# swyoon/Diffusion-by-MaxEntIRL

Hardware: AMD Instinct MI355X
Metric: images/sec (CIFAR-10 DDPM T=10 generation) (higher is better)
Workload: dtype bf16

## Files before the change

diffusion-by-maxentirl_amd/csrc/conv1x1_rw.hip:

```cpp
#include "conv_common.h"
#include <stdlib.h>

namespace {

#define RW_GPTR(p) ((const __attribute__((address_space(1))) void*)(p))
#define RW_LPTR(p) ((__attribute__((address_space(3))) void*)(p))
#define RW_WAIT_VM(n) asm volatile("s_waitcnt vmcnt(%0)" ::"n"(n) : "memory")
__device__ __forceinline__ void rw_barrier() { asm volatile("s_waitcnt lgkmcnt(0)\n\ts_barrier" ::: "memory"); }

constexpr int RW_CHUNK = 64 * 256;
constexpr int RW_RO = 64 * 256;

template <int NCH, int R, bool RES>
__global__ __launch_bounds__(256, ((NCH > 3 || R > 4) ? 1 : 2)) void conv1x1_rw_kernel(ConvArgs p) {
    static_assert(R - 1 <= 4 * NCH && R >= 3 && 4 * (R - 2) + 4 * (RES ? 8 : 4) < 64, "ring depth");
    constexpr int BOPS = RES ? 8 : 4;
    constexpr int NYOUNG = 4 * (R - 2);
    extern __shared__ __attribute__((aligned(1024))) char smem[];
    char* const ring = smem;

    const int tid = threadIdx.x, lane = tid & 63, h = lane >> 5;
    const int wave = __builtin_amdgcn_readfirstlane(tid >> 6);
    char* const ro = smem + R * RW_CHUNK + wave * 4096;
    const int xcd = blockIdx.x & 7, j = blockIdx.x >> 3;
    const int cot = j % p.CT;
    const int nstreams = (gridDim.x >> 3) / p.CT * 8;
    const int stream = (j / p.CT) * 8 + xcd;
    const int ntiles = stream < p.PT ? (p.PT - stream + nstreams - 1) / nstreams : 0;
    if (ntiles == 0) return;

    bf16x8 A[NCH * 8];
    {
        const bf16x8* wf = reinterpret_cast<const bf16x8*>(p.w) + (size_t)(cot * 4 + wave) * 64 + lane;
#pragma unroll
        for (int ks = 0; ks < NCH * 8; ++ks) A[ks] = wf[(size_t)ks * p.CB * 64];
    }
    f32x4 bv[4];
#pragma unroll
// ... 5 lines not shown
    const float slope = dxmi_act_slope(p.act);

    int dpx[4], ds8[4];
#pragma unroll
    for (int u = 0; u < 4; ++u) {
        dpx[u] = (wave * 4 + u) * 4 + (lane >> 4);
        ds8[u] = ((lane & 15) ^ (dpx[u] & 15)) * 8;
    }
    auto issue_chunk = [&](int tile, int c, int slot) {
        const size_t P0 = (size_t)(stream + tile * nstreams) * 64;
        const int cbase = c * 128;
        const bool first = cbase < p.C0;
        const bf16* src = first ? p.in0 : p.in1;
        const int Cs = first ? p.C0 : p.C1;
        const int coff = first ? cbase : cbase - p.C0;
#pragma unroll
        for (int u = 0; u < 4; ++u)
            __builtin_amdgcn_global_load_lds(RW_GPTR(src + (P0 + dpx[u]) * Cs + coff + ds8[u]),
                                             RW_LPTR(ring + slot * RW_CHUNK + (wave * 4 + u) * 1024), 16, 0, 0);
    };
    int rpx[4], rc8[4];
#pragma unroll
    for (int i = 0; i < 4; ++i) {
        rpx[i] = i * 16 + (lane >> 2);
        rc8[i] = ((lane & 3) ^ ((rpx[i] >> 1) & 3)) * 8;
    }
    auto tile_off = [&](int tile, int i) -> size_t {
        return ((size_t)(stream + tile * nstreams) * 64 + rpx[i]) * p.Cout + cot * 128 + wave * 32 + rc8[i];
    };
    auto issue_residual = [&](int tile) {
// ... 3 lines not shown
    };

    const int gtot = ntiles * NCH;
    if (RES) issue_residual(0);
#pragma unroll
    for (int g = 0; g < R - 1; ++g)
        if (g < gtot) issue_chunk(g / NCH, g % NCH, g);

    int boff[8];
    {
        const int px = lane & 31;
#pragma unroll
        for (int ks = 0; ks < 8; ++ks) boff[ks] = px * 256 + (((ks * 2 + h) ^ (px & 15)) << 4);
    }

    int slot = 0;
    for (int ti = 0; ti < ntiles; ++ti) {
        f32x16 acc[2];
#pragma unroll
        for (int nb = 0; nb < 2; ++nb)
#pragma unroll
            for (int r = 0; r < 16; ++r) acc[nb][r] = 0.f;
#pragma unroll
        for (int c = 0; c < NCH; ++c) {
            const int g = ti * NCH + c;
            const int kmax = R - 1 - c > 0 ? (R - 1 - c + NCH - 1) / NCH : 0;
            const int nbnd = ti < kmax ? ti : kmax;
            if (g + R - 2 >= gtot) RW_WAIT_VM(0);
            else if (nbnd == 0) RW_WAIT_VM(NYOUNG);
            else if (nbnd == 1) RW_WAIT_VM(NYOUNG + BOPS);
            else if (nbnd == 2) RW_WAIT_VM(NYOUNG + 2 * BOPS);
            else if (nbnd == 3) RW_WAIT_VM(NYOUNG + 3 * BOPS);
            else RW_WAIT_VM(NYOUNG + 4 * BOPS);
            rw_barrier();
            {
                const int gi = g + R - 1;
                const int si = slot == 0 ? R - 1 : slot - 1;
                if (gi < gtot) issue_chunk(ti + (c + R - 1) / NCH, (c + R - 1) % NCH, si);
            }
            const char* img = ring + slot * RW_CHUNK;
#pragma unroll
            for (int ks = 0; ks < 8; ++ks)
#pragma unroll
                for (int nb = 0; nb < 2; ++nb) {
                    const bf16x8 b = *reinterpret_cast<const bf16x8*>(img + boff[ks] + nb * (32 * 256));
                    acc[nb] = __builtin_amdgcn_mfma_f32_32x32x16_bf16(A[c * 8 + ks], b, acc[nb], 0, 0, 0);
                }
            slot = slot + 1 == R ? 0 : slot + 1;
        }
        if (RES) {
            if ((ti + 1) * NCH + R - 1 > gtot) RW_WAIT_VM(0);
            else RW_WAIT_VM(4 * NCH);
        }
#pragma unroll
        for (int nb = 0; nb < 2; ++nb) {
            const int px = nb * 32 + (lane & 31);
#pragma unroll
            for (int g4 = 0; g4 < 4; ++g4) {
                char* a = ro + px * 64 + ((g4 ^ ((px >> 1) & 3)) << 4) + 8 * h;
                f32x4 v;
#pragma unroll
                for (int e = 0; e < 4; ++e) v[e] = acc[nb][4 * g4 + e] + bv[g4][e];
// ... 13 lines not shown
            bf16x8 v[4];
#pragma unroll
            for (int i = 0; i < 4; ++i) v[i] = *reinterpret_cast<const bf16x8*>(ro + i * 1024 + lane * 16);
#pragma unroll
            for (int i = 0; i < 4; ++i) *reinterpret_cast<bf16x8*>(reinterpret_cast<bf16*>(p.out) + tile_off(ti, i)) = v[i];
        }
        if (RES && ti + 1 < ntiles) issue_residual(ti + 1);
    }
}

template <int NCH, int R>
int rw_launch(const ConvArgs& b, int grid, hipStream_t st) {
    const size_t lds = (size_t)R * RW_CHUNK + RW_RO;
    static bool attr_set = false;
    if (!attr_set) {
        (void)hipFuncSetAttribute(reinterpret_cast<const void*>(conv1x1_rw_kernel<NCH, R, true>), hipFuncAttributeMaxDynamicSharedMemorySize, 160 * 1024);
        (void)hipFuncSetAttribute(reinterpret_cast<const void*>(conv1x1_rw_kernel<NCH, R, false>), hipFuncAttributeMaxDynamicSharedMemorySize, 160 * 1024);
        attr_set = true;
    }
    if (b.residual) hipLaunchKernelGGL((conv1x1_rw_kernel<NCH, R, true>), dim3(grid), dim3(256), lds, st, b);
    else hipLaunchKernelGGL((conv1x1_rw_kernel<NCH, R, false>), dim3(grid), dim3(256), lds, st, b);
    DXMI_CHECK_LAUNCH("dxmi_conv2d_fwd(1x1 rw)");
    return DXMI_OK;
}

}

int conv1x1_rw_try_launch(ConvArgs& a, hipStream_t st, int* kernel_id) {
    static const int enabled = getenv("DXMI_CONV1X1_RW") ? atoi(getenv("DXMI_CONV1X1_RW")) : 1;
    if (!enabled) return 1;
    if (a.in_mode != DXMI_IN_NHWC_BF16 || a.out_mode != DXMI_OUT_NHWC_BF16) return 1;
    if (a.ksize != 1 || a.stride != 1 || a.pad != 0 || a.ups != 0 || a.mask_src || a.addvec || a.act == DXMI_ACT_SILU) return 1;
    const int K = a.C0 + a.C1;
    if (K % 128 != 0 || a.C0 % 128 != 0 || K > 512 || a.Cout % 128 != 0) return 1;
    const long px = (long)a.N * a.OH * a.OW;
    if (px % 64 != 0 || px / 64 < 512) return 1;
    if (kernel_id) {
        const int nch = K / 128;
        *kernel_id = 500000 + nch * 1000 + (nch > 3 ? 6 : 3) * 10 + (a.residual ? 1 : 0);
        return DXMI_OK;
    }
    ConvArgs b = a;
    b.PT = (int)(px / 64);
    b.CT = a.Cout / 128;
    b.tile_px = 64;
    if (b.CT > 32) return 1;
    const int per_xcd = K > 384 ? 32 : 64;
    const int grid = 8 * b.CT * (per_xcd / b.CT);
    switch (K / 128) {
    case 1: return rw_launch<1, 3>(b, grid, st);
    case 2: return rw_launch<2, 3>(b, grid, st);
    case 3: return rw_launch<3, 3>(b, grid, st);
    default: return rw_launch<4, 6>(b, grid, st);
    }
}
```

diffusion-by-maxentirl_amd/csrc/groupnorm.hip:

```cpp
#include "conv_common.h"
#include <stdlib.h>

namespace {

__device__ __forceinline__ int xcd_logical_block(int b, int G, int on = 1) {
    if (!on) return b;
    const int x = b & 7, k = b >> 3;
    const int q = G >> 3, r = G & 7;
    return x * q + (x < r ? x : r) + k;
}

struct GnArgs {
    const bf16* in0;
    const bf16* in1;
    const float* gamma;
    const float* beta;
    bf16* out;
    int C0, C1, HW, groups, slices, ppp, cpg, gps;
    int xcd;
    float eps;
    int silu;
    int fast;
};

// ... 276 lines not shown
struct GnApplyArgs {
    const bf16* in0;
    const bf16* in1;
    const float* st0;
    const float* st1;
    const float* gamma;
    const float* beta;
    const float* ss;
    bf16* out;
    int C0, C1, HW, groups, cpg, chunks, rows_per_chunk, P0, P1, ss_ld;
    float eps;
    int silu;
    int nt;
    float* ab;
};

constexpr int GN_APPLY_MAXP = 8;

typedef int gn_i4 __attribute__((ext_vector_type(4)));
__device__ __forceinline__ bf16x8 gn_ld(const bf16* ptr, bool nt) {
    const gn_i4* q = reinterpret_cast<const gn_i4*>(ptr);
    const gn_i4 t = nt ? __builtin_nontemporal_load(q) : *q;
    return __builtin_bit_cast(bf16x8, t);
}
__device__ __forceinline__ void gn_st(bf16* ptr, const bf16x8& v, bool nt) {
    gn_i4* q = reinterpret_cast<gn_i4*>(ptr);
    const gn_i4 t = __builtin_bit_cast(gn_i4, v);
    if (nt) __builtin_nontemporal_store(t, q);
    else *q = t;
}

template <int U>
// ... 20 lines not shown
        for (int u = 0; u < U; ++u) {
            const int rr = r + u * rows_par;
            if (rr < row1) v[u] = gn_ld(src + (size_t)rr * Cs, p.nt & 1);
        }
    }
    float A[8], Bv[8];
    if (p.ab) {
        if (!active) return;
        const f32x4* q = reinterpret_cast<const f32x4*>(p.ab + ((size_t)n * C + c) * 2);
        const f32x4 t0 = q[0], t1 = q[1], t2 = q[2], t3 = q[3];
        A[0] = t0[0]; Bv[0] = t0[1]; A[1] = t0[2]; Bv[1] = t0[3];
        A[2] = t1[0]; Bv[2] = t1[1]; A[3] = t1[2]; Bv[3] = t1[3];
        A[4] = t2[0]; Bv[4] = t2[1]; A[5] = t2[2]; Bv[5] = t2[3];
        A[6] = t3[0]; Bv[6] = t3[1]; A[7] = t3[2]; Bv[7] = t3[3];
    } else {
    auto pair_sums = [&](const float* st, int P, int nbs, int off) {
        const float2* const base = reinterpret_cast<const float2*>(st) + (size_t)n * P * nbs;
        for (int b = tid; b < nbs; b += 256) {
            float2 t[GN_APPLY_MAXP];
#pragma unroll
            for (int k = 0; k < GN_APPLY_MAXP; ++k)
                if (k < P) t[k] = base[(unsigned)(k * nbs + b)];
            float s = 0.f, q = 0.f;
#pragma unroll
            for (int k = 0; k < GN_APPLY_MAXP; ++k)
                if (k < P) {
                    s += t[k].x;
                    q += t[k].y;
                }
            for (int k = GN_APPLY_MAXP; k < P; ++k) {
                const float2 tk = base[(unsigned)(k * nbs + b)];
                s += tk.x;
                q += tk.y;
            }
            pair_s[off + b] = make_float2(s, q);
        }
    };
    pair_sums(p.st0, p.P0, p.C0 >> 1, 0);
    if (p.C1) pair_sums(p.st1, p.P1, p.C1 >> 1, p.C0 >> 1);
    __syncthreads();
    f32x4 g0, g1, b0, b1;
    if (active) {
        g0 = *reinterpret_cast<const f32x4*>(p.gamma + c);
        g1 = *reinterpret_cast<const f32x4*>(p.gamma + c + 4);
        b0 = *reinterpret_cast<const f32x4*>(p.beta + c);
        b1 = *reinterpret_cast<const f32x4*>(p.beta + c + 4);
    }
    f32x4 sc0 = {0.f, 0.f, 0.f, 0.f}, sc1 = sc0, sh0 = sc0, sh1 = sc0;
    if (active && p.ss) {
        const float* ssn = p.ss + (size_t)n * p.ss_ld + c;
        sc0 = *reinterpret_cast<const f32x4*>(ssn);
        sc1 = *reinterpret_cast<const f32x4*>(ssn + 4);
        sh0 = *reinterpret_cast<const f32x4*>(ssn + C);
        sh1 = *reinterpret_cast<const f32x4*>(ssn + C + 4);
    }
    if (tid < p.groups) {
        const int bpg = p.cpg >> 1;
        float s = 0.f, q = 0.f;
        for (int b = tid * bpg; b < (tid + 1) * bpg; ++b) {
            s += pair_s[b].x;
            q += pair_s[b].y;
        }
        const float cnt = (float)p.HW * (float)p.cpg;
        const float m = s / cnt;
        mean_s[tid] = m;
        rstd_s[tid] = rsqrtf(fmaxf(q / cnt - m * m, 0.f) + p.eps);
    }
    __syncthreads();
    if (!active) return;
    {
#pragma unroll
        for (int e = 0; e < 8; ++e) {
            const int g = (c + e) / p.cpg;
            float a = rstd_s[g] * (e < 4 ? g0[e] : g1[e - 4]);
            float b = (e < 4 ? b0[e] : b1[e - 4]) - mean_s[g] * a;
            if (p.ss) {
                const float sc = 1.f + (e < 4 ? sc0[e] : sc1[e - 4]);
                a *= sc;
                b = b * sc + (e < 4 ? sh0[e] : sh1[e - 4]);
            }
            A[e] = a;
            Bv[e] = b;
        }
    }
    }
    for (;;) {
#pragma unroll
        for (int u = 0; u < U; ++u) {
            const int rr = r + u * rows_par;
            if (rr < row1) {
                bf16x8 o;
#pragma unroll
                for (int e = 0; e < 8; ++e) {
                    float y = (float)v[u][e] * A[e] + Bv[e];
                    if (p.silu) y = dxmi_silu_fast(y);
                    o[e] = (bf16)y;
                }
                gn_st(dst + (size_t)rr * C, o, p.nt & 2);
            }
        }
        r += U * rows_par;
        if (r >= row1) break;
#pragma unroll
        for (int u = 0; u < U; ++u) {
            const int rr = r + u * rows_par;
            if (rr < row1) v[u] = gn_ld(src + (size_t)rr * Cs, p.nt & 1);
        }
    }
}

__global__ __launch_bounds__(256) void gn_block_stats_kernel(const bf16* __restrict__ x, float* __restrict__ st, int HW, int C,
                                                             int chunks, int rows_per_chunk) {
    __shared__ float sm[256 * 8];
// ... 966 lines not shown

extern "C" int dxmi_groupnorm_generic_bwd(const void* in0, int32_t C0, const void* in1, int32_t C1, const void* dy,
                                          const void* add0, const void* add1, const float* gamma, const float* beta,
                                          const float* scale_shift, int32_t ss_ld, void* dx0, void* dx1, float* g_out,
                                          void* workspace, int32_t N, int32_t HW, int32_t groups, float eps,
                                          int32_t apply_silu, void* stream) {
    return dxmi_groupnorm_generic_bwd_saved(in0, C0, in1, C1, dy, add0, add1, gamma, beta, scale_shift, ss_ld, dx0, dx1, g_out, nullptr,
                                            workspace, N, HW, groups, eps, apply_silu, stream);
}

__global__ __launch_bounds__(256) void gn_finalize_kernel(GnApplyArgs p) {
    __shared__ float mean_s[32], rstd_s[32];
    __shared__ float2 pair_s[1024];
    const int C = p.C0 + p.C1;
    const int n = blockIdx.x, tid = threadIdx.x;
    auto pair_sums = [&](const float* st, int P, int nbs, int off) {
        const float2* const base = reinterpret_cast<const float2*>(st) + (size_t)n * P * nbs;
        for (int b = tid; b < nbs; b += 256) {
            float2 t[GN_APPLY_MAXP];
#pragma unroll
            for (int k = 0; k < GN_APPLY_MAXP; ++k)
                if (k < P) t[k] = base[(unsigned)(k * nbs + b)];
            float s = 0.f, q = 0.f;
#pragma unroll
            for (int k = 0; k < GN_APPLY_MAXP; ++k)
                if (k < P) {
                    s += t[k].x;
                    q += t[k].y;
                }
            for (int k = GN_APPLY_MAXP; k < P; ++k) {
                const float2 tk = base[(unsigned)(k * nbs + b)];
                s += tk.x;
                q += tk.y;
            }
            pair_s[off + b] = make_float2(s, q);
        }
    };
    pair_sums(p.st0, p.P0, p.C0 >> 1, 0);
    if (p.C1) pair_sums(p.st1, p.P1, p.C1 >> 1, p.C0 >> 1);
    __syncthreads();
    if (tid < p.groups) {
        const int bpg = p.cpg >> 1;
        float s = 0.f, q = 0.f;
        for (int b = tid * bpg; b < (tid + 1) * bpg; ++b) {
            s += pair_s[b].x;
            q += pair_s[b].y;
        }
        const float cnt = (float)p.HW * (float)p.cpg;
        const float m = s / cnt;
        mean_s[tid] = m;
        rstd_s[tid] = rsqrtf(fmaxf(q / cnt - m * m, 0.f) + p.eps);
    }
    __syncthreads();
    for (int c = tid; c < C; c += 256) {
        const int g = c / p.cpg;
        float a = rstd_s[g] * p.gamma[c];
        float b = p.beta[c] - mean_s[g] * a;
        if (p.ss) {
            const float sc = 1.f + p.ss[(size_t)n * p.ss_ld + c];
            a *= sc;
            b = b * sc + p.ss[(size_t)n * p.ss_ld + C + c];
        }
        reinterpret_cast<float2*>(p.ab)[(size_t)n * C + c] = make_float2(a, b);
    }
}

__global__ __launch_bounds__(256) void gn_blockstats_to_generic_kernel(const float* __restrict__ st0, int P0, int C0, const float* __restrict__ st1,
                                                                      int P1, int C1, float* __restrict__ part, int groups, int chunks) {
    __shared__ float2 pair_s[1024];
    const int n = blockIdx.x, tid = threadIdx.x;
    const int C = C0 + C1, cpg = C / groups;
    auto pair_sums = [&](const float* st, int P, int nbs, int off) {
        const float2* const base = reinterpret_cast<const float2*>(st) + (size_t)n * P * nbs;
        for (int b = tid; b < nbs; b += 256) {
            float s = 0.f, q = 0.f;
            for (int k = 0; k < P; ++k) {
                const float2 t = base[(size_t)k * nbs + b];
// ... 144 lines not shown
    int rpc = trips_env * U * rows_par;
    if (rpc > HW) rpc = HW;
    a.chunks = (HW + rpc - 1) / rpc;
    a.rows_per_chunk = rpc;
    a.ab = ab;
    if (ab) {
        hipLaunchKernelGGL(gn_finalize_kernel, dim3(N), dim3(256), 0, (hipStream_t)stream, a);
        DXMI_CHECK_LAUNCH("dxmi_groupnorm_apply_split(finalize)");
    }
    if (U == 8) hipLaunchKernelGGL(gn_apply_kernel<8>, dim3(N * a.chunks), dim3(256), 0, (hipStream_t)stream, a);
    else if (U == 2) hipLaunchKernelGGL(gn_apply_kernel<2>, dim3(N * a.chunks), dim3(256), 0, (hipStream_t)stream, a);
    else hipLaunchKernelGGL(gn_apply_kernel<4>, dim3(N * a.chunks), dim3(256), 0, (hipStream_t)stream, a);
    DXMI_CHECK_LAUNCH("dxmi_groupnorm_apply");
    return DXMI_OK;
}
```

diffusion-by-maxentirl_amd/dxmi_hip/_lib.py:

```python
import ctypes
import os

_HERE = os.path.dirname(os.path.abspath(__file__))
LIB_PATH = os.environ.get("DXMI_LIB") or os.path.join(_HERE, "libdxmi_hip.so")

c_void_p, c_int, c_float, c_int64 = ctypes.c_void_p, ctypes.c_int32, ctypes.c_float, ctypes.c_int64


class ConvDesc(ctypes.Structure):

    _fields_ = [
        ("in0", c_void_p), ("in1", c_void_p), ("wpacked", c_void_p), ("bias", c_void_p),
        ("addvec", c_void_p), ("residual", c_void_p), ("out", c_void_p),
        ("N", c_int), ("IH", c_int), ("IW", c_int), ("C0", c_int), ("C1", c_int),
        ("OH", c_int), ("OW", c_int), ("Cout", c_int),
        ("ksize", c_int), ("stride", c_int), ("pad", c_int), ("upsample", c_int), ("act", c_int),
        ("addvec_ld", c_int), ("in_mode", c_int), ("out_mode", c_int), ("variant", c_int),
        ("mask_src", c_void_p), ("mask_slope", c_float), ("gn_stats", c_void_p),
        ("gn_out", c_void_p), ("gn_gamma", c_void_p), ("gn_beta", c_void_p), ("gn_eps", c_float), ("gn_groups", c_int), ("gn_flags", c_int),
    ]


class PackItem(ctypes.Structure):

# ... 7 lines not shown
    "dxmi_device_check": (c_int, []),
    "dxmi_set_tuning": (c_int, [ctypes.c_char_p, c_int]),
    "dxmi_get_tuning": (c_int, [ctypes.c_char_p, ctypes.POINTER(c_int)]),
    "dxmi_conv2d_fwd": (c_int, [ctypes.POINTER(ConvDesc), c_void_p]),
    "dxmi_conv2d_kernel_id": (c_int, [ctypes.POINTER(ConvDesc)]),
    "dxmi_conv2d_gn_stats_partials": (c_int, [ctypes.POINTER(ConvDesc)]),
    "dxmi_conv2d_gn_fuse_supported": (c_int, [ctypes.POINTER(ConvDesc)]),
    "dxmi_conv_ws_last_clock": (c_int, [ctypes.POINTER(ctypes.c_uint64)]),
    "dxmi_gn_block_stats_partials": (c_int, [c_int]),
    "dxmi_gn_block_stats": (c_int, [c_void_p, c_void_p, c_int, c_int, c_int, c_void_p]),
    "dxmi_gn_stats_fold": (c_int, [c_void_p, c_void_p, c_int, c_int, c_int, c_int, c_void_p]),
    "dxmi_groupnorm_apply": (c_int, [c_void_p, c_int, c_void_p, c_int, c_void_p, c_int, c_void_p, c_int, c_void_p, c_void_p, c_void_p, c_int,
                                     c_void_p, c_int, c_int, c_int, c_float, c_int, c_void_p]),
    "dxmi_groupnorm_apply_split": (c_int, [c_void_p, c_int, c_void_p, c_int, c_void_p, c_int, c_void_p, c_int, c_void_p, c_void_p, c_void_p, c_int,
                                           c_void_p, c_void_p, c_int, c_int, c_int, c_float, c_int, c_void_p]),
    "dxmi_gn_blockstats_to_generic": (c_int, [c_void_p, c_int, c_int, c_void_p, c_int, c_int, c_void_p, c_int, c_int, c_int, c_void_p]),
    "dxmi_attention_fwd_lse_supported": (c_int, [c_int, c_int, c_int]),
    "dxmi_attention_fwd_lse": (c_int, [c_void_p, c_void_p, c_void_p, c_int, c_int, c_int, c_int, c_float, c_void_p]),
    "dxmi_attention_bwd_lse": (c_int, [c_void_p, c_void_p, c_void_p, c_void_p, c_void_p, c_void_p, c_int, c_int, c_int, c_int, c_float, c_void_p]),
    "dxmi_gn_ss_grads": (c_int, [c_void_p, c_void_p, c_int, c_void_p, c_void_p, c_void_p, c_void_p, c_void_p, c_int, c_int, c_void_p]),
    "dxmi_fid_stats_workspace_bytes": (c_int64, [c_int64, c_int]),
    "dxmi_fid_stats": (c_int, [c_void_p, c_int64, c_int, c_void_p, c_void_p, c_void_p, c_void_p]),
    "dxmi_knn_radii_workspace_bytes": (c_int64, [c_int64, c_int, c_int, c_int]),
    "dxmi_knn_radii": (c_int, [c_void_p, c_int64, c_int, c_int, c_int, c_void_p, c_void_p, c_void_p]),
    "dxmi_pr_membership_workspace_bytes": (c_int64, [c_int64, c_int64]),
    "dxmi_pr_membership": (c_int, [c_void_p, c_int64, c_void_p, c_void_p, c_int64, c_void_p, c_int, c_void_p, c_void_p, c_void_p, c_void_p]),
    "dxmi_inception_score_workspace_bytes": (c_int64, [c_int64, c_int, c_int]),
    "dxmi_inception_score": (c_int, [c_void_p, c_int64, c_int, c_void_p, c_int, c_int, c_void_p, c_void_p, c_void_p]),
    "dxmi_packed_conv_weight_bytes": (c_int64, [c_int, c_int, c_int, c_int]),
    "dxmi_pack_conv_weights": (c_int, [ctypes.POINTER(PackItem), c_int, c_void_p]),
# ... 102 lines not shown
```

diffusion-by-maxentirl_amd/dxmi_hip/ops.py:

```python
import ctypes
import os

import torch

from . import _lib
from . import graph as _graph
from ._lib import ConvDesc, check, load

ACT_NONE, ACT_LEAKY02, ACT_RELU, ACT_SILU = 0, 1, 2, 3
IN_NHWC_BF16, IN_NCHW_F32_K27 = 0, 1
OUT_NHWC_BF16, OUT_NCHW_F32 = 0, 1


_RAW_STREAM = getattr(torch._C, "_cuda_getCurrentRawStream", None)
_GET_DEVICE = getattr(torch._C, "_cuda_getDevice", None)


def _stream():
    if _RAW_STREAM is not None and _GET_DEVICE is not None:
        return ctypes.c_void_p(_RAW_STREAM(_GET_DEVICE()))
    return ctypes.c_void_p(torch.cuda.current_stream().cuda_stream)


def _tree_fingerprint(module):
# ... 664 lines not shown
            saved.append(gn_blockstats_to_generic(stats[0], stats[1] if in1 is not None else None, N, H * W, C0, C1, groups))
        return groupnorm_apply(x, stats[0], gamma, beta, in1=in1, st1=stats[1] if in1 is not None else None, groups=groups,
                               eps=eps, silu=silu, out=out, scale_shift=scale_shift)
    if scale_shift is not None or not load().dxmi_groupnorm_silu_supported(C0, C1, H * W, groups):
        return groupnorm_generic(x, gamma, beta, in1=in1, groups=groups, eps=eps, silu=silu, out=out, scale_shift=scale_shift, saved=saved)
    assert x.dtype == torch.bfloat16 and x.is_contiguous()
    assert gamma.dtype == torch.float32 and beta.dtype == torch.float32 and gamma.numel() == C0 + C1
    if out is None:
        out = torch.empty((N, H, W, C0 + C1), dtype=torch.bfloat16, device=x.device)
    _prof("groupnorm", "resident", 0.0, 4.0 * N * H * W * (C0 + C1), lambda: check(
        load().dxmi_groupnorm_silu_fwd(_ptr(x), C0, _ptr(in1), C1, _ptr(gamma), _ptr(beta), _ptr(out), N, H * W,
                                       groups, float(eps), int(silu), _stream()), "dxmi_groupnorm_silu_fwd"))
    return out


def gn_blockstats_to_generic(st0, st1, N, HW, C0, C1, groups=32):
    lib = load()
    ws = torch.empty(lib.dxmi_groupnorm_generic_workspace_bytes(N, HW, C0 + C1) // 4, dtype=torch.float32, device=st0.buf.device)
    check(lib.dxmi_gn_blockstats_to_generic(_ptr(st0.buf), st0.P, C0, _ptr(st1.buf) if st1 is not None else None, st1.P if st1 is not None else 0,
                                            C1, _ptr(ws), N, HW, groups, _stream()), "dxmi_gn_blockstats_to_generic")
    return ws


def groupnorm_generic(x, gamma, beta, *, in1=None, groups=32, eps=1e-5, silu=True, out=None, scale_shift=None, saved=None):
    _need_cuda(x, in1, gamma, beta, out, scale_shift)
    N, H, W, C0 = x.shape
    C1 = in1.shape[3] if in1 is not None else 0
    C = C0 + C1
    assert x.dtype == torch.bfloat16 and x.is_contiguous()
    if out is None:
# ... 616 lines not shown
```

diffusion-by-maxentirl_amd/models/DxMI/unet_small.py:

```python
import torch
import torch.nn as nn

from dxmi_hip import ops
from dxmi_hip._lib import DxmiError


def Normalize(in_channels):
    return nn.GroupNorm(num_groups=32, num_channels=in_channels, eps=1e-6, affine=True)


def _conv(cin, cout, k, stride=1, padding=0):
    return nn.Conv2d(cin, cout, kernel_size=k, stride=stride, padding=padding)


class Upsample(nn.Module):

    def __init__(self, in_channels, with_conv):
        super().__init__()
        self.with_conv = with_conv
        if with_conv:
            self.conv = _conv(in_channels, in_channels, 3, 1, 1)


class Downsample(nn.Module):
# ... 183 lines not shown
        return self._packed

    def refresh_packs(self):
        self.packed()
        if getattr(self, "_packed_t", None) is not None:
            from .unet_small_train import _pack_t
            _pack_t(self)

    def prepare_capture(self):
        if getattr(self, "_packed_t", None) is not None:
            for k in [k for k in self._packed_t if k not in self._packed_t_planned]:
                del self._packed_t[k]
        self.refresh_packs()

    FUSE_ATTN_PROJ = True
    FUSE_ATTN_BLOCK = True
    FUSE_GN_SMALL = True
    STREAM_GN_MIN_HW = 256

    def _conv_s(self, x, pw, **kw):
        out, st = ops.conv2d(x, pw, want_stats=True, **kw)
        if st is None and out.shape[1] * out.shape[2] >= self.STREAM_GN_MIN_HW:
            st = ops.block_stats(out)
        return out, st

    def _resblock(self, pk, b, x0, x1, tp, s0=None, s1=None, nxt=None):
        if isinstance(s0, _Normed):
            assert s0.norm is b.norm1 and x1 is None
            a0 = s0.y
        else:
            a0 = ops.groupnorm_silu(x0, b.norm1.weight, b.norm1.bias, in1=x1, eps=1e-6, silu=True, stats=(s0, s1))
        off = pk[id(b), "toff"]
        stream = x0.shape[1] * x0.shape[2] >= self.STREAM_GN_MIN_HW
        a = None
        if not stream and self.FUSE_GN_SMALL:
            h, a = ops.conv2d(a0, pk[id(b), "conv1"], bias=b.conv1.bias, addvec=tp[:, off:off + b.out_channels],
                              fuse_gn=(b.norm2.weight, b.norm2.bias, 32, 1e-6, True, False))
            sh = None
            if a is None and stream:
                sh = ops.block_stats(h)
        else:
            h, sh = ops.conv2d(a0, pk[id(b), "conv1"], bias=b.conv1.bias, addvec=tp[:, off:off + b.out_channels], want_stats=True)
        if a is None:
            a = ops.groupnorm_silu(h, b.norm2.weight, b.norm2.bias, eps=1e-6, silu=True, stats=(sh, None))
        if b.in_channels != b.out_channels:
            sc_mod = b.conv_shortcut if b.use_conv_shortcut else b.nin_shortcut
            sc = ops.conv2d(x0, pk[id(b), "short"], in1=x1, bias=sc_mod.bias)
        else:
            assert x1 is None
            sc = x0
        if stream:
            return self._conv_s(a, pk[id(b), "conv2"], bias=b.conv2.bias, residual=sc)
        if nxt is not None and self.FUSE_GN_SMALL:
            h, y = ops.conv2d(a, pk[id(b), "conv2"], bias=b.conv2.bias, residual=sc,
                              fuse_gn=(nxt[0].weight, nxt[0].bias, 32, 1e-6, nxt[1], True))
            return h, (None if y is None else _Normed(y, nxt[0]))
        return ops.conv2d(a, pk[id(b), "conv2"], bias=b.conv2.bias, residual=sc), None

    def _attn(self, pk, m, x, sx=None):
        N, H, W, C = x.shape
        if self.FUSE_ATTN_BLOCK and (id(m), "block") in pk and isinstance(sx, ops.BlockStats) and ops.attn_block_supported(H * W, C, 1):
            return ops.attn_block(x, sx, m.norm.weight, m.norm.bias, pk[id(m), "block"], eps=1e-6, want_stats=True)
# ... 98 lines not shown
```

include/dxmi_hip.h:

```cpp
#ifndef DXMI_HIP_H
#define DXMI_HIP_H

#include <stdint.h>

#ifdef __cplusplus
extern "C" {
#endif

#define DXMI_OK            0
#define DXMI_EINVAL       -1
#define DXMI_ELAUNCH      -2
#define DXMI_ENODEV       -3

#define DXMI_ACT_NONE      0
#define DXMI_ACT_LEAKY02   1
#define DXMI_ACT_RELU      2
#define DXMI_ACT_SILU      3

#define DXMI_IN_NHWC_BF16     0
#define DXMI_IN_NCHW_F32_K27  1
#define DXMI_IN_ROWS_F32      2
#define DXMI_OUT_NHWC_BF16    0
#define DXMI_OUT_NCHW_F32     1
#define DXMI_OUT_ROWS_F32     2
// ... 115 lines not shown
                            int32_t apply_silu, void* stream);

int dxmi_gn_block_stats_partials(int32_t HW);
int dxmi_gn_block_stats(const void* x, float* stats, int32_t N, int32_t HW, int32_t C, void* stream);
int dxmi_gn_stats_fold(const float* stats, float* out, int32_t N, int32_t P, int32_t C, int32_t group, void* stream);
int dxmi_groupnorm_apply(const void* in0, int32_t C0, const float* stats0, int32_t P0, const void* in1, int32_t C1,
                         const float* stats1, int32_t P1, const float* gamma, const float* beta, const float* scale_shift,
                         int32_t ss_ld, void* out, int32_t N, int32_t HW, int32_t groups, float eps, int32_t apply_silu,
                         void* stream);

int dxmi_groupnorm_apply_split(const void* in0, int32_t C0, const float* stats0, int32_t P0, const void* in1, int32_t C1,
                               const float* stats1, int32_t P1, const float* gamma, const float* beta,
                               const float* scale_shift, int32_t ss_ld, void* out, float* ab_workspace, int32_t N, int32_t HW,
                               int32_t groups, float eps, int32_t apply_silu, void* stream);

int dxmi_gn_blockstats_to_generic(const float* stats0, int32_t P0, int32_t C0, const float* stats1, int32_t P1, int32_t C1,
                                  float* generic_stats, int32_t N, int32_t HW, int32_t groups, void* stream);

int dxmi_gn_ss_grads(const float* g, const float* scale_shift, int32_t ss_ld, const float* gamma, const float* beta,
                     float* d_scale_shift, float* dgamma, float* dbeta, int32_t N, int32_t C, void* stream);

int dxmi_attention_fwd(const void* qkv, void* out, int32_t N, int32_t T, int32_t C,
                       int32_t heads, float scale, void* stream);

int dxmi_attention_proj_supported(int32_t T, int32_t C, int32_t heads);
int dxmi_pack_attn_proj_weight(const float* w_oi, void* dst, void* stream);
int dxmi_attention_proj_fwd(const void* qkv, const void* wproj_packed, const float* bias, const void* residual, void* out,
                            float* gn_stats, int32_t N, int32_t T, int32_t C, int32_t heads, float scale, void* stream);

int dxmi_attn_block_supported(int32_t T, int32_t C, int32_t heads, int32_t groups);
// ... 188 lines not shown
```

Baseline: 6733.

## Fuse GroupNorm+SiLU apply into the 1x1 shortcut conv kernel

Adds a GN variant of the 1x1 streaming conv kernel. While computing the nin_shortcut it normalizes the staged input chunks already in LDS and writes the GroupNorm+SiLU output as a side result. Per-image scale/shift tables are loaded into LDS alongside each chunk, and vmcnt waits are recomputed through a runtime switch. The resblock path uses it when channels change at large spatial sizes, so the input is read once instead of twice. The cost is an extra gn_finalize launch, more LDS, extra stores inside the MFMA loop, and more complex wait-count bookkeeping.

```diff
diff --git a/diffusion-by-maxentirl_amd/csrc/conv1x1_rw.hip b/diffusion-by-maxentirl_amd/csrc/conv1x1_rw.hip
--- a/diffusion-by-maxentirl_amd/csrc/conv1x1_rw.hip
+++ b/diffusion-by-maxentirl_amd/csrc/conv1x1_rw.hip
@@ -1,4 +1,5 @@
 #include "conv_common.h"
+#include "gn_common.h"
 #include <stdlib.h>
 
 namespace {
@@ -10,10 +11,29 @@
 
 constexpr int RW_CHUNK = 64 * 256;
 constexpr int RW_RO = 64 * 256;
-
-template <int NCH, int R, bool RES>
-__global__ __launch_bounds__(256, ((NCH > 3 || R > 4) ? 1 : 2)) void conv1x1_rw_kernel(ConvArgs p) {
+constexpr int RW_TBL = 128 * 8;
+
+struct RwGn {
+    const float* ab;
+    bf16* y;
+    int HW, silu;
+};
+
+__device__ __forceinline__ void rw_wait_vm(int n) {
+    switch (__builtin_amdgcn_readfirstlane(n)) {
+#define RW_C(k) case k: RW_WAIT_VM(k); break;
+#define RW_C8(k) RW_C(k) RW_C(k + 1) RW_C(k + 2) RW_C(k + 3) RW_C(k + 4) RW_C(k + 5) RW_C(k + 6) RW_C(k + 7)
+    RW_C8(0) RW_C8(8) RW_C8(16) RW_C8(24) RW_C8(32) RW_C8(40) RW_C8(48) RW_C8(56)
+#undef RW_C8
+#undef RW_C
+    default: RW_WAIT_VM(0);
+    }
+}
+
+template <int NCH, int R, bool RES, bool GN>
+__global__ __launch_bounds__(256, ((NCH > 3 || R > 4) ? 1 : 2)) void conv1x1_rw_kernel(ConvArgs p, RwGn q) {
     static_assert(R - 1 <= 4 * NCH && R >= 3 && 4 * (R - 2) + 4 * (RES ? 8 : 4) < 64, "ring depth");
+    static_assert(!(GN && RES) && (!GN || 5 * (R - 2) + 4 * 4 + 4 * (R - 1) < 64), "GN side output: no residual, vmcnt range");
     constexpr int BOPS = RES ? 8 : 4;
     constexpr int NYOUNG = 4 * (R - 2);
     extern __shared__ __attribute__((aligned(1024))) char smem[];
@@ -22,6 +42,7 @@
     const int tid = threadIdx.x, lane = tid & 63, h = lane >> 5;
     const int wave = __builtin_amdgcn_readfirstlane(tid >> 6);
     char* const ro = smem + R * RW_CHUNK + wave * 4096;
+    char* const tbl = smem + R * RW_CHUNK + RW_RO;
     const int xcd = blockIdx.x & 7, j = blockIdx.x >> 3;
     const int cot = j % p.CT;
     const int nstreams = (gridDim.x >> 3) / p.CT * 8;
@@ -57,6 +78,11 @@
         const bf16* src = first ? p.in0 : p.in1;
         const int Cs = first ? p.C0 : p.C1;
         const int coff = first ? cbase : cbase - p.C0;
+        if constexpr (GN) {
+            const int n = (int)P0 / q.HW;
+            __builtin_amdgcn_global_load_lds(RW_GPTR(q.ab + ((size_t)n * (NCH * 128) + cbase) * 2 + wave * 64 + lane),
+                                             RW_LPTR(tbl + slot * RW_TBL + wave * 256), 4, 0, 0);
+        }
 #pragma unroll
         for (int u = 0; u < 4; ++u)
             __builtin_amdgcn_global_load_lds(RW_GPTR(src + (P0 + dpx[u]) * Cs + coff + ds8[u]),
@@ -90,6 +116,9 @@
         for (int ks = 0; ks < 8; ++ks) boff[ks] = px * 256 + (((ks * 2 + h) ^ (px & 15)) << 4);
     }
 
+    const int gnp = GN ? 4 / p.CT : 0;
+    const int gs = tid & 15, gpx0 = cot * (64 / p.CT) + (tid >> 4);
+
     int slot = 0;
     for (int ti = 0; ti < ntiles; ++ti) {
         f32x16 acc[2];
@@ -103,6 +132,7 @@
             const int kmax = R - 1 - c > 0 ? (R - 1 - c + NCH - 1) / NCH : 0;
             const int nbnd = ti < kmax ? ti : kmax;
             if (g + R - 2 >= gtot) RW_WAIT_VM(0);
+            else if (GN) rw_wait_vm(5 * (R - 2) + nbnd * BOPS + (g < R - 1 ? g : R - 1) * gnp);
             else if (nbnd == 0) RW_WAIT_VM(NYOUNG);
             else if (nbnd == 1) RW_WAIT_VM(NYOUNG + BOPS);
             else if (nbnd == 2) RW_WAIT_VM(NYOUNG + 2 * BOPS);
@@ -122,6 +152,21 @@
                     const bf16x8 b = *reinterpret_cast<const bf16x8*>(img + boff[ks] + nb * (32 * 256));
                     acc[nb] = __builtin_amdgcn_mfma_f32_32x32x16_bf16(A[c * 8 + ks], b, acc[nb], 0, 0, 0);
                 }
+            if constexpr (GN) {
+                float ga[8], gb[8];
+                const f32x4* t = reinterpret_cast<const f32x4*>(tbl + slot * RW_TBL + gs * 64);
+#pragma unroll
+                for (int i = 0; i < 4; ++i) {
+                    const f32x4 v = t[i];
+                    ga[2 * i] = v[0]; gb[2 * i] = v[1]; ga[2 * i + 1] = v[2]; gb[2 * i + 1] = v[3];
+                }
+                bf16* const yt = q.y + (size_t)(stream + ti * nstreams) * 64 * (NCH * 128) + c * 128 + gs * 8;
+                for (int i = 0; i < gnp; ++i) {
+                    const int px = gpx0 + 16 * i;
+                    const bf16x8 v = *reinterpret_cast<const bf16x8*>(img + px * 256 + ((gs ^ (px & 15)) << 4));
+                    *reinterpret_cast<bf16x8*>(yt + (size_t)px * (NCH * 128)) = gn_norm8(v, ga, gb, q.silu);
+                }
+            }
             slot = slot + 1 == R ? 0 : slot + 1;
         }
         if (RES) {
@@ -165,14 +210,37 @@
     const size_t lds = (size_t)R * RW_CHUNK + RW_RO;
     static bool attr_set = false;
     if (!attr_set) {
-        (void)hipFuncSetAttribute(reinterpret_cast<const void*>(conv1x1_rw_kernel<NCH, R, true>), hipFuncAttributeMaxDynamicSharedMemorySize, 160 * 1024);
-        (void)hipFuncSetAttribute(reinterpret_cast<const void*>(conv1x1_rw_kernel<NCH, R, false>), hipFuncAttributeMaxDynamicSharedMemorySize, 160 * 1024);
+        (void)hipFuncSetAttribute(reinterpret_cast<const void*>(conv1x1_rw_kernel<NCH, R, true, false>), hipFuncAttributeMaxDynamicSharedMemorySize, 160 * 1024);
+        (void)hipFuncSetAttribute(reinterpret_cast<const void*>(conv1x1_rw_kernel<NCH, R, false, false>), hipFuncAttributeMaxDynamicSharedMemorySize, 160 * 1024);
         attr_set = true;
     }
-    if (b.residual) hipLaunchKernelGGL((conv1x1_rw_kernel<NCH, R, true>), dim3(grid), dim3(256), lds, st, b);
-    else hipLaunchKernelGGL((conv1x1_rw_kernel<NCH, R, false>), dim3(grid), dim3(256), lds, st, b);
+    const RwGn none = {};
+    if (b.residual) hipLaunchKernelGGL((conv1x1_rw_kernel<NCH, R, true, false>), dim3(grid), dim3(256), lds, st, b, none);
+    else hipLaunchKernelGGL((conv1x1_rw_kernel<NCH, R, false, false>), dim3(grid), dim3(256), lds, st, b, none);
     DXMI_CHECK_LAUNCH("dxmi_conv2d_fwd(1x1 rw)");
     return DXMI_OK;
+}
+
+template <int NCH, int R>
+int rw_launch_gn(const ConvArgs& b, const RwGn& g, int grid, hipStream_t st) {
+    const size_t lds = (size_t)R * (RW_CHUNK + RW_TBL) + RW_RO;
+    static bool attr_set = false;
+    if (!attr_set) {
+        (void)hipFuncSetAttribute(reinterpret_cast<const void*>(conv1x1_rw_kernel<NCH, R, false, true>), hipFuncAttributeMaxDynamicSharedMemorySize, 160 * 1024);
+        attr_set = true;
+    }
+    hipLaunchKernelGGL((conv1x1_rw_kernel<NCH, R, false, true>), dim3(grid), dim3(256), lds, st, b, g);
+    DXMI_CHECK_LAUNCH("dxmi_groupnorm_silu_shortcut");
+    return DXMI_OK;
+}
+
+int rw_grid(ConvArgs& b) {
+    const int K = b.C0 + b.C1;
+    b.PT = (int)((long)b.N * b.OH * b.OW / 64);
+    b.CT = b.Cout / 128;
+    b.tile_px = 64;
+    const int per_xcd = K > 384 ? 32 : 64;
+    return 8 * b.CT * (per_xcd / b.CT);
 }
 
 }
@@ -192,12 +260,8 @@
         return DXMI_OK;
     }
     ConvArgs b = a;
-    b.PT = (int)(px / 64);
-    b.CT = a.Cout / 128;
-    b.tile_px = 64;
-    if (b.CT > 32) return 1;
-    const int per_xcd = K > 384 ? 32 : 64;
-    const int grid = 8 * b.CT * (per_xcd / b.CT);
+    if (a.Cout / 128 > 32) return 1;
+    const int grid = rw_grid(b);
     switch (K / 128) {
     case 1: return rw_launch<1, 3>(b, grid, st);
     case 2: return rw_launch<2, 3>(b, grid, st);
@@ -205,3 +269,48 @@
     default: return rw_launch<4, 6>(b, grid, st);
     }
 }
+
+static int gn_shortcut_nch(const dxmi_conv_desc* d, int groups) {
+    if (!d || d->ksize != 1 || d->stride != 1 || d->pad != 0 || d->upsample || d->residual || d->addvec || d->mask_src || d->gn_stats ||
+        d->gn_out || d->act != DXMI_ACT_NONE || d->variant != 0 || d->in_mode != DXMI_IN_NHWC_BF16 || d->out_mode != DXMI_OUT_NHWC_BF16)
+        return 0;
+    const int K = d->C0 + d->C1, CT = d->Cout / 128;
+    if (d->IH != d->OH || d->IW != d->OW || (d->OH * d->OW) % 64 != 0) return 0;
+    if (CT != 1 && CT != 2 && CT != 4) return 0;
+    if (groups <= 0 || groups > 32 || K % groups != 0 || (K / groups) % 2 != 0 || d->C1 % 8 != 0) return 0;
+    const int id = dxmi_conv2d_kernel_id(d);
+    const int nch = K / 128;
+    if (K % 128 != 0 || nch < 1 || nch > 4 || id != 500000 + nch * 1000 + (nch > 3 ? 6 : 3) * 10) return 0;
+    return nch;
+}
+
+extern "C" int dxmi_groupnorm_silu_shortcut_supported(const dxmi_conv_desc* d, int32_t groups) {
+    return gn_shortcut_nch(d, groups) > 0 ? 1 : 0;
+}
+
+extern "C" int dxmi_groupnorm_silu_shortcut(const dxmi_conv_desc* d, const float* stats0, int32_t P0, const float* stats1, int32_t P1,
+                                            const float* gamma, const float* beta, int32_t groups, float eps, int32_t apply_silu, void* y,
+                                            float* ab_workspace, void* stream) {
+    DXMI_CHECK_ARG(d && d->in0 && d->wpacked && d->out && y && ab_workspace && stats0 && gamma && beta && P0 > 0,
+                   "dxmi_groupnorm_silu_shortcut: null pointer");
+    DXMI_CHECK_ARG(d->C1 == 0 || (d->in1 && stats1 && P1 > 0), "dxmi_groupnorm_silu_shortcut: C1>0 needs in1 and stats1");
+    const int nch = gn_shortcut_nch(d, groups);
+    if (nch == 0) return 1;
+    const int HW = d->OH * d->OW;
+    int rc = gn_finalize_launch(stats0, P0, d->C0, stats1, P1, d->C1, gamma, beta, ab_workspace, d->N, HW, groups, eps, (hipStream_t)stream);
+    if (rc != DXMI_OK) return rc;
+    ConvArgs b = {};
+    b.in0 = (const bf16*)d->in0; b.in1 = (const bf16*)d->in1; b.w = (const bf16*)d->wpacked; b.bias = d->bias; b.out = d->out;
+    b.N = d->N; b.IH = d->IH; b.IW = d->IW; b.C0 = d->C0; b.C1 = d->C1; b.OH = d->OH; b.OW = d->OW; b.Cout = d->Cout;
+    b.ksize = 1; b.stride = 1; b.act = DXMI_ACT_NONE; b.in_mode = DXMI_IN_NHWC_BF16; b.out_mode = DXMI_OUT_NHWC_BF16;
+    b.CB = (d->Cout + 31) / 32;
+    const int grid = rw_grid(b);
+    const RwGn g = {ab_workspace, (bf16*)y, HW, apply_silu ? 1 : 0};
+    const hipStream_t st = (hipStream_t)stream;
+    switch (nch) {
+    case 1: return rw_launch_gn<1, 3>(b, g, grid, st);
+    case 2: return rw_launch_gn<2, 3>(b, g, grid, st);
+    case 3: return rw_launch_gn<3, 3>(b, g, grid, st);
+    default: return rw_launch_gn<4, 6>(b, g, grid, st);
+    }
+}
diff --git a/diffusion-by-maxentirl_amd/csrc/gn_common.h b/diffusion-by-maxentirl_amd/csrc/gn_common.h
--- /dev/null
+++ b/diffusion-by-maxentirl_amd/csrc/gn_common.h
@@ -0,0 +1,64 @@
+#pragma once
+#include "common.h"
+
+constexpr int GN_APPLY_MAXP = 8;
+
+__device__ __forceinline__ void gn_pair_sums(float2* pair_s, const float* st, int n, int P, int nbs, int off, int tid) {
+    const float2* const base = reinterpret_cast<const float2*>(st) + (size_t)n * P * nbs;
+    for (int b = tid; b < nbs; b += 256) {
+        float2 t[GN_APPLY_MAXP];
+#pragma unroll
+        for (int k = 0; k < GN_APPLY_MAXP; ++k)
+            if (k < P) t[k] = base[(unsigned)(k * nbs + b)];
+        float s = 0.f, q = 0.f;
+#pragma unroll
+        for (int k = 0; k < GN_APPLY_MAXP; ++k)
+            if (k < P) {
+                s += t[k].x;
+                q += t[k].y;
+            }
+        for (int k = GN_APPLY_MAXP; k < P; ++k) {
+            const float2 tk = base[(unsigned)(k * nbs + b)];
+            s += tk.x;
+            q += tk.y;
+        }
+        pair_s[off + b] = make_float2(s, q);
+    }
+}
+
+__device__ __forceinline__ void gn_group_moments(const float2* pair_s, int g, int cpg, int HW, float eps, float* mean_s, float* rstd_s) {
+    const int bpg = cpg >> 1;
+    float s = 0.f, q = 0.f;
+    for (int b = g * bpg; b < (g + 1) * bpg; ++b) {
+        s += pair_s[b].x;
+        q += pair_s[b].y;
+    }
+    const float cnt = (float)HW * (float)cpg;
+    const float m = s / cnt;
+    mean_s[g] = m;
+    rstd_s[g] = rsqrtf(fmaxf(q / cnt - m * m, 0.f) + eps);
+}
+
+__device__ __forceinline__ void gn_channel_ab(float mean, float rstd, float gamma, float beta, float& a, float& b) {
+    a = rstd * gamma;
+    b = beta - mean * a;
+}
+__device__ __forceinline__ void gn_film(float& a, float& b, float scale, float shift) {
+    const float sc = 1.f + scale;
+    a *= sc;
+    b = b * sc + shift;
+}
+
+__device__ __forceinline__ bf16x8 gn_norm8(const bf16x8& v, const float* A, const float* B, int silu) {
+    bf16x8 o;
+#pragma unroll
+    for (int e = 0; e < 8; ++e) {
+        float y = (float)v[e] * A[e] + B[e];
+        if (silu) y = dxmi_silu_fast(y);
+        o[e] = (bf16)y;
+    }
+    return o;
+}
+
+int gn_finalize_launch(const float* stats0, int P0, int C0, const float* stats1, int P1, int C1, const float* gamma, const float* beta,
+                       float* ab, int N, int HW, int groups, float eps, hipStream_t st);
diff --git a/diffusion-by-maxentirl_amd/csrc/groupnorm.hip b/diffusion-by-maxentirl_amd/csrc/groupnorm.hip
--- a/diffusion-by-maxentirl_amd/csrc/groupnorm.hip
+++ b/diffusion-by-maxentirl_amd/csrc/groupnorm.hip
@@ -1,4 +1,5 @@
 #include "conv_common.h"
+#include "gn_common.h"
 #include <stdlib.h>
 
 namespace {
@@ -314,8 +315,6 @@
     int nt;
     float* ab;
 };
-
-constexpr int GN_APPLY_MAXP = 8;
 
 typedef int gn_i4 __attribute__((ext_vector_type(4)));
 __device__ __forceinline__ bf16x8 gn_ld(const bf16* ptr, bool nt) {
@@ -366,30 +365,8 @@
         A[4] = t2[0]; Bv[4] = t2[1]; A[5] = t2[2]; Bv[5] = t2[3];
         A[6] = t3[0]; Bv[6] = t3[1]; A[7] = t3[2]; Bv[7] = t3[3];
     } else {
-    auto pair_sums = [&](const float* st, int P, int nbs, int off) {
-        const float2* const base = reinterpret_cast<const float2*>(st) + (size_t)n * P * nbs;
-        for (int b = tid; b < nbs; b += 256) {
-            float2 t[GN_APPLY_MAXP];
-#pragma unroll
-            for (int k = 0; k < GN_APPLY_MAXP; ++k)
-                if (k < P) t[k] = base[(unsigned)(k * nbs + b)];
-            float s = 0.f, q = 0.f;
-#pragma unroll
-            for (int k = 0; k < GN_APPLY_MAXP; ++k)
-                if (k < P) {
-                    s += t[k].x;
-                    q += t[k].y;
-                }
-            for (int k = GN_APPLY_MAXP; k < P; ++k) {
-                const float2 tk = base[(unsigned)(k * nbs + b)];
-                s += tk.x;
-                q += tk.y;
-            }
-            pair_s[off + b] = make_float2(s, q);
-        }
-    };
-    pair_sums(p.st0, p.P0, p.C0 >> 1, 0);
-    if (p.C1) pair_sums(p.st1, p.P1, p.C1 >> 1, p.C0 >> 1);
+    gn_pair_sums(pair_s, p.st0, n, p.P0, p.C0 >> 1, 0, tid);
+    if (p.C1) gn_pair_sums(pair_s, p.st1, n, p.P1, p.C1 >> 1, p.C0 >> 1, tid);
     __syncthreads();
     f32x4 g0, g1, b0, b1;
     if (active) {
@@ -406,33 +383,15 @@
         sh0 = *reinterpret_cast<const f32x4*>(ssn + C);
         sh1 = *reinterpret_cast<const f32x4*>(ssn + C + 4);
     }
-    if (tid < p.groups) {
-        const int bpg = p.cpg >> 1;
-        float s = 0.f, q = 0.f;
-        for (int b = tid * bpg; b < (tid + 1) * bpg; ++b) {
-            s += pair_s[b].x;
-            q += pair_s[b].y;
-        }
-        const float cnt = (float)p.HW * (float)p.cpg;
-        const float m = s / cnt;
-        mean_s[tid] = m;
-        rstd_s[tid] = rsqrtf(fmaxf(q / cnt - m * m, 0.f) + p.eps);
-    }
+    if (tid < p.groups) gn_group_moments(pair_s, tid, p.cpg, p.HW, p.eps, mean_s, rstd_s);
     __syncthreads();
     if (!active) return;
     {
 #pragma unroll
         for (int e = 0; e < 8; ++e) {
             const int g = (c + e) / p.cpg;
-            float a = rstd_s[g] * (e < 4 ? g0[e] : g1[e - 4]);
-            float b = (e < 4 ? b0[e] : b1[e - 4]) - mean_s[g] * a;
-            if (p.ss) {
-                const float sc = 1.f + (e < 4 ? sc0[e] : sc1[e - 4]);
-                a *= sc;
-                b = b * sc + (e < 4 ? sh0[e] : sh1[e - 4]);
-            }
-            A[e] = a;
-            Bv[e] = b;
+            gn_channel_ab(mean_s[g], rstd_s[g], e < 4 ? g0[e] : g1[e - 4], e < 4 ? b0[e] : b1[e - 4], A[e], Bv[e]);
+            if (p.ss) gn_film(A[e], Bv[e], e < 4 ? sc0[e] : sc1[e - 4], e < 4 ? sh0[e] : sh1[e - 4]);
         }
     }
     }
@@ -441,14 +400,7 @@
         for (int u = 0; u < U; ++u) {
             const int rr = r + u * rows_par;
             if (rr < row1) {
-                bf16x8 o;
-#pragma unroll
-                for (int e = 0; e < 8; ++e) {
-                    float y = (float)v[u][e] * A[e] + Bv[e];
-                    if (p.silu) y = dxmi_silu_fast(y);
-                    o[e] = (bf16)y;
-                }
-                gn_st(dst + (size_t)rr * C, o, p.nt & 2);
+                gn_st(dst + (size_t)rr * C, gn_norm8(v[u], A, Bv, p.silu), p.nt & 2);
             }
         }
         r += U * rows_par;
@@ -1445,53 +1397,16 @@
     __shared__ float2 pair_s[1024];
     const int C = p.C0 + p.C1;
     const int n = blockIdx.x, tid = threadIdx.x;
-    auto pair_sums = [&](const float* st, int P, int nbs, int off) {
-        const float2* const base = reinterpret_cast<const float2*>(st) + (size_t)n * P * nbs;
-        for (int b = tid; b < nbs; b += 256) {
-            float2 t[GN_APPLY_MAXP];
-#pragma unroll
-            for (int k = 0; k < GN_APPLY_MAXP; ++k)
-                if (k < P) t[k] = base[(unsigned)(k * nbs + b)];
-            float s = 0.f, q = 0.f;
-#pragma unroll
-            for (int k = 0; k < GN_APPLY_MAXP; ++k)
-                if (k < P) {
-                    s += t[k].x;
-                    q += t[k].y;
-                }
-            for (int k = GN_APPLY_MAXP; k < P; ++k) {
-                const float2 tk = base[(unsigned)(k * nbs + b)];
-                s += tk.x;
-                q += tk.y;
-            }
-            pair_s[off + b] = make_float2(s, q);
-        }
-    };
-    pair_sums(p.st0, p.P0, p.C0 >> 1, 0);
-    if (p.C1) pair_sums(p.st1, p.P1, p.C1 >> 1, p.C0 >> 1);
-    __syncthreads();
-    if (tid < p.groups) {
-        const int bpg = p.cpg >> 1;
-        float s = 0.f, q = 0.f;
-        for (int b = tid * bpg; b < (tid + 1) * bpg; ++b) {
-            s += pair_s[b].x;
-            q += pair_s[b].y;
-        }
-        const float cnt = (float)p.HW * (float)p.cpg;
-        const float m = s / cnt;
-        mean_s[tid] = m;
-        rstd_s[tid] = rsqrtf(fmaxf(q / cnt - m * m, 0.f) + p.eps);
-    }
+    gn_pair_sums(pair_s, p.st0, n, p.P0, p.C0 >> 1, 0, tid);
+    if (p.C1) gn_pair_sums(pair_s, p.st1, n, p.P1, p.C1 >> 1, p.C0 >> 1, tid);
+    __syncthreads();
+    if (tid < p.groups) gn_group_moments(pair_s, tid, p.cpg, p.HW, p.eps, mean_s, rstd_s);
     __syncthreads();
     for (int c = tid; c < C; c += 256) {
         const int g = c / p.cpg;
-        float a = rstd_s[g] * p.gamma[c];
-        float b = p.beta[c] - mean_s[g] * a;
-        if (p.ss) {
-            const float sc = 1.f + p.ss[(size_t)n * p.ss_ld + c];
-            a *= sc;
-            b = b * sc + p.ss[(size_t)n * p.ss_ld + C + c];
-        }
+        float a, b;
+        gn_channel_ab(mean_s[g], rstd_s[g], p.gamma[c], p.beta[c], a, b);
+        if (p.ss) gn_film(a, b, p.ss[(size_t)n * p.ss_ld + c], p.ss[(size_t)n * p.ss_ld + C + c]);
         reinterpret_cast<float2*>(p.ab)[(size_t)n * C + c] = make_float2(a, b);
     }
 }
@@ -1666,3 +1581,18 @@
     DXMI_CHECK_LAUNCH("dxmi_groupnorm_apply");
     return DXMI_OK;
 }
+
+int gn_finalize_launch(const float* stats0, int P0, int C0, const float* stats1, int P1, int C1, const float* gamma, const float* beta,
+                       float* ab, int N, int HW, int groups, float eps, hipStream_t st) {
+    DXMI_CHECK_ARG(stats0 && gamma && beta && ab && P0 > 0 && N > 0 && HW > 0, "gn_finalize: null pointer / empty shape");
+    DXMI_CHECK_ARG(C1 == 0 || (stats1 && P1 > 0), "gn_finalize: C1>0 needs stats1");
+    const int C = C0 + C1;
+    DXMI_CHECK_ARG(groups > 0 && groups <= 32 && C % groups == 0 && (C / groups) % 2 == 0 && C0 % 8 == 0 && C1 % 8 == 0 && C <= 2048,
+                   "gn_finalize: C0=%d C1=%d groups=%d (even channels per group)", C0, C1, groups);
+    GnApplyArgs a = {};
+    a.st0 = stats0; a.st1 = stats1; a.gamma = gamma; a.beta = beta; a.ss = nullptr; a.ab = ab;
+    a.C0 = C0; a.C1 = C1; a.HW = HW; a.groups = groups; a.cpg = C / groups; a.P0 = P0; a.P1 = P1; a.eps = eps;
+    hipLaunchKernelGGL(gn_finalize_kernel, dim3(N), dim3(256), 0, st, a);
+    DXMI_CHECK_LAUNCH("gn_finalize");
+    return DXMI_OK;
+}
diff --git a/diffusion-by-maxentirl_amd/dxmi_hip/_lib.py b/diffusion-by-maxentirl_amd/dxmi_hip/_lib.py
--- a/diffusion-by-maxentirl_amd/dxmi_hip/_lib.py
+++ b/diffusion-by-maxentirl_amd/dxmi_hip/_lib.py
@@ -45,6 +45,9 @@
                                      c_void_p, c_int, c_int, c_int, c_float, c_int, c_void_p]),
     "dxmi_groupnorm_apply_split": (c_int, [c_void_p, c_int, c_void_p, c_int, c_void_p, c_int, c_void_p, c_int, c_void_p, c_void_p, c_void_p, c_int,
                                            c_void_p, c_void_p, c_int, c_int, c_int, c_float, c_int, c_void_p]),
+    "dxmi_groupnorm_silu_shortcut_supported": (c_int, [ctypes.POINTER(ConvDesc), c_int]),
+    "dxmi_groupnorm_silu_shortcut": (c_int, [ctypes.POINTER(ConvDesc), c_void_p, c_int, c_void_p, c_int, c_void_p, c_void_p, c_int, c_float,
+                                             c_int, c_void_p, c_void_p, c_void_p]),
     "dxmi_gn_blockstats_to_generic": (c_int, [c_void_p, c_int, c_int, c_void_p, c_int, c_int, c_void_p, c_int, c_int, c_int, c_void_p]),
     "dxmi_attention_fwd_lse_supported": (c_int, [c_int, c_int, c_int]),
     "dxmi_attention_fwd_lse": (c_int, [c_void_p, c_void_p, c_void_p, c_int, c_int, c_int, c_int, c_float, c_void_p]),
diff --git a/diffusion-by-maxentirl_amd/dxmi_hip/ops.py b/diffusion-by-maxentirl_amd/dxmi_hip/ops.py
--- a/diffusion-by-maxentirl_amd/dxmi_hip/ops.py
+++ b/diffusion-by-maxentirl_amd/dxmi_hip/ops.py
@@ -702,6 +702,46 @@
     return out
 
 
+def groupnorm_silu_shortcut(x, gamma, beta, pw, *, in1=None, bias=None, groups=32, eps=1e-6, silu=True, stats=None):
+    _need_cuda(x, in1, gamma, beta, bias)
+    if stats is None or stats[0] is None or (in1 is not None and stats[1] is None) or pw.k27 or pw.ksize != 1:
+        return None
+    N, H, W, C0 = x.shape
+    C1 = in1.shape[3] if in1 is not None else 0
+    C = C0 + C1
+    if (C // groups) % 2 != 0 or C0 % 8 != 0 or C1 % 8 != 0:
+        return None
+    assert x.dtype == torch.bfloat16 and x.is_contiguous() and C == pw.Cin
+    assert in1 is None or (in1.dtype == torch.bfloat16 and in1.is_contiguous() and in1.shape[:3] == x.shape[:3])
+    assert gamma.dtype == torch.float32 and beta.dtype == torch.float32 and gamma.numel() == C and beta.numel() == C
+    st0, st1 = stats[0], (stats[1] if in1 is not None else None)
+    assert tuple(st0.buf.shape) == (N, st0.P, C0 // 2, 2) and (st1 is None or tuple(st1.buf.shape) == (N, st1.P, C1 // 2, 2))
+    Cout = pw.Cout
+    sc = torch.empty((N, H, W, Cout), dtype=torch.bfloat16, device=x.device)
+    d = ConvDesc()
+    d.in0, d.in1, d.wpacked = x.data_ptr(), (in1.data_ptr() if in1 is not None else None), pw.buf.data_ptr()
+    d.bias = bias.data_ptr() if bias is not None else None
+    d.out = sc.data_ptr()
+    d.N, d.IH, d.IW, d.C0, d.C1, d.OH, d.OW, d.Cout = N, H, W, C0, C1, H, W, Cout
+    d.ksize, d.stride, d.pad, d.upsample, d.act = 1, 1, 0, 0, ACT_NONE
+    d.in_mode, d.out_mode = IN_NHWC_BF16, OUT_NHWC_BF16
+    lib = load()
+    key = ("gn_shortcut", N, H, W, C0, C1, Cout, groups, bias is not None)
+    ok = _STATS_P.get(key)
+    if ok is None:
+        ok = _STATS_P[key] = int(lib.dxmi_groupnorm_silu_shortcut_supported(ctypes.byref(d), groups))
+    if not ok:
+        return None
+    y = torch.empty((N, H, W, C), dtype=torch.bfloat16, device=x.device)
+    ab = torch.empty((N, C, 2), dtype=torch.float32, device=x.device)
+    px = N * H * W
+    _prof("groupnorm", "gn_shortcut", 2.0 * px * C * Cout, 2.0 * (2 * px * C + px * Cout + C * Cout), lambda: check(
+        lib.dxmi_groupnorm_silu_shortcut(ctypes.byref(d), _ptr(st0.buf), st0.P, _ptr(st1.buf) if st1 is not None else None,
+                                         st1.P if st1 is not None else 0, _ptr(gamma), _ptr(beta), groups, float(eps), int(silu),
+                                         _ptr(y), _ptr(ab), _stream()), "dxmi_groupnorm_silu_shortcut"))
+    return y, sc
+
+
 def gn_blockstats_to_generic(st0, st1, N, HW, C0, C1, groups=32):
     lib = load()
     ws = torch.empty(lib.dxmi_groupnorm_generic_workspace_bytes(N, HW, C0 + C1) // 4, dtype=torch.float32, device=st0.buf.device)
diff --git a/diffusion-by-maxentirl_amd/models/DxMI/unet_small.py b/diffusion-by-maxentirl_amd/models/DxMI/unet_small.py
--- a/diffusion-by-maxentirl_amd/models/DxMI/unet_small.py
+++ b/diffusion-by-maxentirl_amd/models/DxMI/unet_small.py
@@ -1,3 +1,5 @@
+import os
+
 import torch
 import torch.nn as nn
 
@@ -221,6 +223,7 @@
         self.refresh_packs()
 
     FUSE_ATTN_PROJ = True
+    FUSE_GN_SHORTCUT = os.environ.get("DXMI_GN_SHORTCUT", "1") != "0"
     FUSE_ATTN_BLOCK = True
     FUSE_GN_SMALL = True
     STREAM_GN_MIN_HW = 256
@@ -232,13 +235,20 @@
         return out, st
 
     def _resblock(self, pk, b, x0, x1, tp, s0=None, s1=None, nxt=None):
+        stream = x0.shape[1] * x0.shape[2] >= self.STREAM_GN_MIN_HW
+        fused = None
         if isinstance(s0, _Normed):
             assert s0.norm is b.norm1 and x1 is None
             a0 = s0.y
         else:
-            a0 = ops.groupnorm_silu(x0, b.norm1.weight, b.norm1.bias, in1=x1, eps=1e-6, silu=True, stats=(s0, s1))
+            if self.FUSE_GN_SHORTCUT and stream and b.in_channels != b.out_channels and not b.use_conv_shortcut:
+                fused = ops.groupnorm_silu_shortcut(x0, b.norm1.weight, b.norm1.bias, pk[id(b), "short"], in1=x1, bias=b.nin_shortcut.bias,
+                                                    eps=1e-6, silu=True, stats=(s0, s1))
+            if fused is not None:
+                a0, sc = fused
+            else:
+                a0 = ops.groupnorm_silu(x0, b.norm1.weight, b.norm1.bias, in1=x1, eps=1e-6, silu=True, stats=(s0, s1))
         off = pk[id(b), "toff"]
-        stream = x0.shape[1] * x0.shape[2] >= self.STREAM_GN_MIN_HW
         a = None
         if not stream and self.FUSE_GN_SMALL:
             h, a = ops.conv2d(a0, pk[id(b), "conv1"], bias=b.conv1.bias, addvec=tp[:, off:off + b.out_channels],
@@ -251,8 +261,9 @@
         if a is None:
             a = ops.groupnorm_silu(h, b.norm2.weight, b.norm2.bias, eps=1e-6, silu=True, stats=(sh, None))
         if b.in_channels != b.out_channels:
-            sc_mod = b.conv_shortcut if b.use_conv_shortcut else b.nin_shortcut
-            sc = ops.conv2d(x0, pk[id(b), "short"], in1=x1, bias=sc_mod.bias)
+            if fused is None:
+                sc_mod = b.conv_shortcut if b.use_conv_shortcut else b.nin_shortcut
+                sc = ops.conv2d(x0, pk[id(b), "short"], in1=x1, bias=sc_mod.bias)
         else:
             assert x1 is None
             sc = x0
diff --git a/include/dxmi_hip.h b/include/dxmi_hip.h
--- a/include/dxmi_hip.h
+++ b/include/dxmi_hip.h
@@ -153,6 +153,11 @@
                                const float* scale_shift, int32_t ss_ld, void* out, float* ab_workspace, int32_t N, int32_t HW,
                                int32_t groups, float eps, int32_t apply_silu, void* stream);
 
+int dxmi_groupnorm_silu_shortcut_supported(const dxmi_conv_desc* d, int32_t groups);
+int dxmi_groupnorm_silu_shortcut(const dxmi_conv_desc* d, const float* stats0, int32_t P0, const float* stats1, int32_t P1,
+                                 const float* gamma, const float* beta, int32_t groups, float eps, int32_t apply_silu, void* y,
+                                 float* ab_workspace, void* stream);
+
 int dxmi_gn_blockstats_to_generic(const float* stats0, int32_t P0, int32_t C0, const float* stats1, int32_t P1, int32_t C1,
                                   float* generic_stats, int32_t N, int32_t HW, int32_t groups, void* stream);
 
```

Result: faster. 7020, median of 6 (+4.3%).
